# zuston/TonY

Hardware: AMD Instinct MI355X
Metric: images/sec (whole node) Inception-v3 TF-PS (higher is better)
Workload: dtype bf16

## Files before the change

tony_amd/ops/_lib.py:

```python
from __future__ import annotations

import ctypes
import os
import threading
import weakref
from typing import Dict

import torch

_HERE = os.path.dirname(os.path.abspath(__file__))
SO_PATH = os.environ.get("TONY_KERNELS_SO") or os.path.join(_HERE, "_tony_kernels.so")

_lock = threading.Lock()
_lib = None

c_void_p = ctypes.c_void_p
c_int = ctypes.c_int
c_int64 = ctypes.c_int64
c_float = ctypes.c_float
c_int_p = ctypes.POINTER(ctypes.c_int)
c_void_pp = ctypes.POINTER(ctypes.c_void_p)
c_u8_p = ctypes.POINTER(ctypes.c_uint8)
c_u64_p = ctypes.POINTER(ctypes.c_uint64)

_SIGNATURES = {
    "tony_bn_fwd_train": [c_void_p, c_int64, c_int, c_int64, c_void_p, c_int64, c_void_p, c_void_p, c_int,
                          c_float, c_int, c_void_p, c_void_p, c_void_p, c_void_p, c_void_p, c_float, c_void_p],
    "tony_bn_fwd_infer": [c_void_p, c_int64, c_int, c_int64, c_void_p, c_int64, c_void_p, c_void_p, c_int,
                          c_float, c_int, c_void_p, c_void_p, c_void_p],
    "tony_bn_bwd": [c_void_p, c_int64, c_void_p, c_int64, c_void_p, c_int64, c_int64, c_int, c_void_p, c_void_p,
                    c_void_p, c_void_p, c_int, c_int, c_void_p, c_void_p, c_void_p, c_int, c_void_p],
    "tony_stat_shards": [],
    "tony_bn_stats": [c_void_p, c_int64, c_int, c_int64, c_void_p, c_void_p, c_int64, c_void_p],
    "tony_bn_apply": [c_void_p, c_int64, c_int, c_int64, c_void_p, c_int64, c_void_p, c_void_p, c_int64, c_void_p,
                      c_void_p, c_int, c_float, c_int, c_int, c_void_p, c_void_p, c_void_p, c_void_p, c_float,
                      c_void_p],
    "tony_bn_apply_segs": [c_void_p, c_int64, c_int, c_int64, c_int, c_int, c_int, c_int, c_int, c_void_p, c_void_p,
                           c_void_p, c_void_p, c_int64, c_int64, c_int64, c_int64, c_void_p, c_void_p, c_int64,
                           c_void_p, c_void_p, c_int, c_float, c_int, c_int, c_void_p, c_void_p, c_void_p, c_void_p,
                           c_float, c_void_p],
    "tony_bn_bwd_reduce_segs": [c_void_p, c_int64, c_int, c_int, c_int, c_int, c_int, c_void_p, c_void_p, c_void_p,
                                c_void_p, c_int64, c_int64, c_int64, c_int64, c_int64, c_int, c_void_p, c_void_p,
                                c_void_p, c_void_p, c_int, c_int, c_void_p, c_void_p, c_int64, c_void_p],
    "tony_bn_bwd_apply_segs": [c_void_p, c_int64, c_int, c_int, c_int, c_int, c_int, c_void_p, c_void_p, c_void_p,
                               c_void_p, c_int64, c_int64, c_int64, c_int64, c_void_p, c_int64, c_int64, c_int,
                               c_void_p, c_void_p, c_void_p, c_void_p, c_int, c_int, c_void_p, c_void_p, c_int64,
                               c_void_p, c_void_p, c_int, c_void_p],
    "tony_bn_relu_maxpool": [c_void_p, c_int64, c_void_p, c_void_p, c_int64, c_void_p, c_void_p, c_int, c_float,
                             c_void_p, c_void_p, c_void_p, c_void_p, c_float, c_void_p, c_int64, c_void_p, c_int,
                             c_int, c_int, c_int, c_int, c_int, c_int, c_void_p],
    "tony_bn_bwd_reduce": [c_void_p, c_int64, c_void_p, c_int64, c_int64, c_int, c_void_p, c_void_p, c_void_p,
                           c_void_p, c_int, c_int, c_void_p, c_void_p, c_int64, c_void_p],
    "tony_bn_bwd_apply": [c_void_p, c_int64, c_void_p, c_int64, c_void_p, c_int64, c_int64, c_int, c_void_p,
                          c_void_p, c_void_p, c_void_p, c_int, c_int, c_void_p, c_void_p, c_int64, c_void_p,
                          c_void_p, c_int, c_void_p],
    "tony_bn_apply_f32_x3": [c_void_p, c_int64, c_int, c_int64, c_void_p, c_int64, c_void_p, c_void_p, c_int64,
                             c_void_p, c_void_p, c_int, c_float, c_int, c_int, c_void_p, c_void_p, c_void_p, c_void_p,
                             c_float, c_void_p],
    "tony_bn_apply_res": [c_void_p, c_int64, c_int, c_int64, c_void_p, c_int64, c_void_p, c_int64, c_void_p,
                          c_void_p, c_int64, c_void_p, c_void_p, c_int, c_float, c_int, c_int, c_void_p, c_void_p,
                          c_void_p, c_void_p, c_float, c_void_p],
    "tony_bn_apply_res_m": [c_void_p, c_int64, c_int, c_int64, c_void_p, c_int64, c_void_p, c_int64, c_void_p,
                            c_void_p, c_int64, c_void_p, c_void_p, c_int, c_float, c_int, c_int, c_void_p, c_void_p,
                            c_void_p, c_void_p, c_float, c_void_p, c_int64, c_void_p],
    "tony_bn_bwd_res": [c_void_p, c_int64, c_void_p, c_int64, c_void_p, c_int64, c_void_p, c_int64, c_void_p, c_int64,
                        c_int64, c_int, c_void_p, c_void_p, c_void_p, c_void_p, c_int, c_void_p, c_void_p, c_void_p,
                        c_int, c_void_p],
    "tony_bn_bwd_res_m": [c_void_p, c_int64, c_void_p, c_int64, c_void_p, c_int64, c_void_p, c_int64, c_void_p,
                          c_int64, c_int64, c_int, c_void_p, c_void_p, c_void_p, c_void_p, c_int, c_void_p, c_void_p,
                          c_void_p, c_int, c_void_p],
    "tony_bn_bwd_onepass": [c_void_p, c_int64, c_void_p, c_int64, c_void_p, c_int64, c_int64, c_int, c_void_p,
                            c_void_p, c_void_p, c_void_p, c_int, c_int, c_void_p, c_void_p, c_void_p, c_int,
                            c_void_p, c_int, c_void_p],
    "tony_add_f32": [c_void_p, c_int, c_void_p, c_int64, c_void_p],
    "tony_sgd_step": [c_void_p, c_void_p, c_void_p, c_int, c_void_p, c_int64, c_void_p, c_void_p],
    "tony_adam_step": [c_void_p, c_void_p, c_void_p, c_void_p, c_int, c_void_p, c_int64, c_void_p, c_void_p],
    "tony_adagrad_step": [c_void_p, c_void_p, c_void_p, c_int, c_void_p, c_int64, c_void_p, c_void_p],
    "tony_rmsprop_step": [c_void_p, c_void_p, c_void_p, c_void_p, c_int, c_void_p, c_int64, c_void_p, c_void_p],
    "tony_grad_stats": [c_void_p, c_int, c_int64, c_void_p, c_void_p],
    "tony_xent_fwd": [c_void_p, c_int, c_int64, c_int, c_int64, c_void_p, c_float, c_void_p, c_void_p, c_void_p],
    "tony_xent_bwd": [c_void_p, c_int, c_int64, c_int, c_int64, c_void_p, c_float, c_void_p, c_void_p, c_void_p,
                      c_int64, c_void_p],
    "tony_dropout_fwd": [c_void_p, c_void_p, c_void_p, c_int64, c_int, c_float, c_void_p, c_void_p],
    "tony_dropout_bwd": [c_void_p, c_void_p, c_void_p, c_int64, c_int, c_float, c_void_p],
    "tony_counter_bump": [c_void_p, c_void_p],
    "tony_gemm_bf16": [c_void_p, c_void_p, c_void_p, c_int64, c_int64, c_int64, c_int64, c_int64, c_int64,
                       c_int, c_void_p, c_int64, c_void_p],
    "tony_gemm_bf16_bnact": [c_void_p, c_void_p, c_void_p, c_int64, c_int64, c_int64, c_int64, c_int64, c_int64,
                             c_int, c_void_p, c_int64, c_void_p, c_void_p],
    "tony_gemm_tn_bf16": [c_void_p, c_void_p, c_void_p, c_int64, c_int64, c_int64, c_int64, c_int64, c_int64,
                          c_void_p, c_int64, c_void_p, c_int, c_void_p, c_void_p, c_int, c_void_p],
    "tony_splitk_reduce": [c_void_p, c_int, c_int64, c_void_p, c_int, c_int, c_int, c_void_p],
    "tony_splitk_workspace": [c_void_p, c_int64, c_void_p, c_int64],
    "tony_conv_fwd": [c_void_p, c_int, c_int, c_int, c_int, c_int64, c_void_p, c_int, c_int, c_int, c_int, c_int,
                      c_int, c_int, c_void_p, c_int, c_int, c_int64, c_int, c_void_p, c_int64, c_void_p],
    "tony_stem_fwd": [c_void_p, c_int, c_int, c_int, c_int, c_void_p, c_int, c_int, c_int, c_int, c_int, c_int,
                      c_int, c_void_p, c_int, c_int, c_int64, c_int, c_void_p, c_int64, c_int, c_void_p],
    "tony_stem_wgrad": [c_void_p, c_int64, c_void_p, c_int, c_int, c_int, c_int, c_int, c_int, c_int, c_int, c_int,
                        c_int, c_int, c_int, c_int, c_void_p, c_int64, c_void_p, c_int, c_void_p],
    "tony_conv_dgrad": [c_void_p, c_int, c_int, c_int, c_int, c_int64, c_void_p, c_int, c_int, c_int, c_int, c_int,
                        c_void_p, c_int, c_int, c_int64, c_int, c_void_p, c_void_p],
    "tony_conv_dgrad_strided": [c_void_p, c_int, c_int, c_int, c_int, c_int64, c_void_p, c_int, c_int, c_int, c_int,
                                c_int, c_int, c_int, c_void_p, c_int, c_int, c_int64, c_int, c_void_p, c_void_p],
    "tony_conv_wgrad": [c_void_p, c_int64, c_void_p, c_int, c_int, c_int, c_int, c_int64, c_int, c_int, c_int, c_int,
                        c_int, c_int, c_int, c_int, c_int, c_void_p, c_void_p, c_int64, c_void_p, c_int, c_void_p,
                        c_void_p, c_int, c_void_p],
    "tony_conv_wgrad_x3": [c_void_p, c_int64, c_void_p, c_int, c_int, c_int, c_int, c_int64, c_int, c_int, c_int,
                           c_int, c_int, c_int, c_int, c_int, c_int, c_int, c_int, c_void_p, c_int64, c_void_p, c_int,
                           c_void_p],
    "tony_x3_wgrad_mode": [c_int],
    "tony_dgrad_one_launch": [c_int],
    "tony_wgrad_pf": [c_int],
    "tony_kv_copy_blocks": [c_int64],
    "tony_kv_copy_flag": [c_void_p, c_void_p, c_int64, c_void_p, c_void_p],
    "tony_kv_wait": [c_void_p, ctypes.c_uint32, c_void_p, ctypes.c_double, c_void_p],
    "tony_conv_wgrad_direct": [c_void_p, c_int64, c_void_p, c_int, c_int, c_int, c_int, c_int64, c_int, c_int, c_int,
                               c_int, c_int, c_void_p, c_int64, c_void_p, c_int, c_void_p],
    "tony_avgpool3_s1p1": [c_void_p, c_void_p, c_int, c_int, c_int, c_int, c_int64, c_int64, c_void_p],
    "tony_maxpool_fwd": [c_void_p, c_void_p, c_void_p, c_int, c_int, c_int, c_int, c_int, c_int, c_int, c_int64, c_int64,
                         c_void_p],
    "tony_maxpool_bwd": [c_void_p, c_void_p, c_void_p, c_int, c_int, c_int, c_int, c_int, c_int, c_int, c_int64, c_int64,
                         c_void_p],
    "tony_bn_bwd_pool_apply": [c_void_p, c_int64, c_void_p, c_int, c_int, c_int, c_int, c_int, c_int, c_int, c_void_p,
                               c_int64, c_void_p, c_int64, c_void_p, c_void_p, c_void_p, c_void_p, c_int, c_int,
                               c_void_p, c_int64, c_void_p, c_void_p, c_int, c_void_p],
    "tony_maxpool_bwd_acc": [c_void_p, c_void_p, c_void_p, c_int, c_int, c_int, c_int, c_int, c_int, c_int, c_int64, c_int64,
                         c_void_p],
    "tony_maxpool_bwd_bnred": [c_void_p, c_void_p, c_void_p, c_int, c_int, c_int, c_int, c_int, c_int, c_int, c_int64,
                               c_int64, c_void_p, c_int64, c_void_p, c_void_p, c_void_p, c_void_p, c_int, c_int,
                               c_void_p, c_int64, c_int, c_void_p],
    "tony_avgpool_fwd": [c_void_p, c_void_p, c_int, c_int, c_int, c_int, c_int, c_int, c_int64, c_int64, c_void_p],
    "tony_avgpool_bwd": [c_void_p, c_void_p, c_int, c_int, c_int, c_int, c_int, c_int, c_int64, c_int64, c_void_p],
    "tony_transpose_desc_bytes": [],
    "tony_x3_desc_bytes": [],
    "tony_x3_weights_batch": [c_void_p, c_int, c_int, c_void_p],
    "tony_transpose_batch": [c_void_p, c_int, c_int, c_void_p],
    "tony_event_pool": [c_int, c_u64_p],
    "tony_fork": [c_void_p, c_void_p, c_void_p],
    "tony_bn_stats_f32": [c_void_p, c_int64, c_int, c_int64, c_void_p, c_void_p, c_int64, c_void_p],
    "tony_bn_apply_f32": [c_void_p, c_int64, c_int, c_int64, c_void_p, c_int64, c_void_p, c_void_p, c_int64, c_void_p,
                      c_void_p, c_int, c_float, c_int, c_int, c_void_p, c_void_p, c_void_p, c_void_p, c_float,
                      c_void_p],
    "tony_bn_bwd_reduce_f32": [c_void_p, c_int64, c_void_p, c_int64, c_int64, c_int, c_void_p, c_void_p, c_void_p,
                           c_void_p, c_int, c_int, c_void_p, c_void_p, c_int64, c_void_p],
    "tony_bn_bwd_apply_f32": [c_void_p, c_int64, c_void_p, c_int64, c_void_p, c_int64, c_int64, c_int, c_void_p,
                          c_void_p, c_void_p, c_void_p, c_int, c_int, c_void_p, c_void_p, c_int64, c_void_p,
                          c_void_p, c_int, c_void_p],
    "tony_bn_bwd_apply_f32_x3": [c_void_p, c_int64, c_void_p, c_int64, c_void_p, c_int64, c_int64, c_int, c_void_p,
                          c_void_p, c_void_p, c_void_p, c_int, c_int, c_void_p, c_void_p, c_int64, c_void_p,
                          c_void_p, c_int, c_void_p],
    "tony_bn_bwd_apply_f32_x3p": [c_void_p, c_int64, c_void_p, c_int64, c_void_p, c_int64, c_int64, c_int64, c_int,
                                  c_void_p, c_void_p, c_void_p, c_void_p, c_int, c_int, c_void_p, c_void_p, c_int64,
                                  c_void_p, c_void_p, c_int, c_void_p],
    "tony_avgpool3_s1p1_f32": [c_void_p, c_void_p, c_int, c_int, c_int, c_int, c_int64, c_int64, c_void_p],
    "tony_avgpool3_s1p1_x3p": [c_void_p, c_void_p, c_int, c_int, c_int, c_int, c_int64, c_int64, c_int64, c_void_p],
    "tony_avgpool3_s1p1_acc": [c_void_p, c_void_p, c_int, c_int, c_int, c_int, c_int64, c_int64, c_int, c_void_p],
    "tony_avgpool3_s1p1_x3": [c_void_p, c_void_p, c_int, c_int, c_int, c_int, c_int64, c_void_p],
    "tony_maxpool_fwd_f32": [c_void_p, c_void_p, c_void_p, c_int, c_int, c_int, c_int, c_int, c_int, c_int, c_int64, c_int64,
                         c_void_p],
    "tony_maxpool_bwd_f32": [c_void_p, c_void_p, c_void_p, c_int, c_int, c_int, c_int, c_int, c_int, c_int, c_int64, c_int64,
                         c_void_p],
    "tony_maxpool_bwd_acc_f32": [c_void_p, c_void_p, c_void_p, c_int, c_int, c_int, c_int, c_int, c_int, c_int, c_int64, c_int64,
                         c_void_p],
    "tony_avgpool_fwd_f32": [c_void_p, c_void_p, c_int, c_int, c_int, c_int, c_int, c_int, c_int64, c_int64, c_void_p],
    "tony_avgpool_bwd_f32": [c_void_p, c_void_p, c_int, c_int, c_int, c_int, c_int, c_int, c_int64, c_int64, c_void_p],
    "tony_x3_split": [c_void_p, c_int64, c_int64, c_int, c_int, c_void_p, c_int64, c_int, c_void_p],
    "tony_x3_split_slice": [c_void_p, c_int64, c_int64, c_int, c_void_p, c_int64, c_int, c_int, c_void_p],
    "tony_bn_apply_f32_p3": [c_void_p, c_int64, c_int, c_int64, c_void_p, c_int64, c_void_p, c_int64, c_int64,
                             c_void_p, c_void_p, c_int64, c_void_p, c_void_p, c_int, c_float, c_int, c_int, c_void_p,
                             c_void_p, c_void_p, c_void_p, c_float, c_void_p],
    "tony_x3_weights_t": [c_void_p, c_int, c_int, c_int, c_void_p, c_void_p],
    "tony_plan_mark": [c_int, c_void_p],
    "tony_plan_build": [c_void_p, c_u64_p, c_int, c_u64_p, c_int_p],
    "tony_plan_replay": [c_void_p, c_int, c_void_p],
    "tony_plan_segments": [c_void_p],
    "tony_plan_failure": [c_void_p, c_int_p],
    "tony_plan_ops": [c_void_p, c_int_p, c_int],
    "tony_plan_destroy": [c_void_p],
    "tony_ps_header_bytes": [],
    "tony_kv_copy": [c_void_p, c_void_p, c_int64, c_void_p, c_void_p],
    "tony_ps_max_buckets": [],
    "tony_ps_max_blocks": [],
    "tony_ps_land_entry_bytes": [],
    "tony_ps_window_alloc": [c_int64, c_void_pp, c_u8_p],
    "tony_ps_push": [c_void_p, c_int, c_void_p, c_int64, c_int, c_int64, c_int, c_int, ctypes.c_uint32, c_int,
                     c_void_p],
    "tony_ps_apply": [c_void_p, c_int64, c_int64, c_int, c_int, c_int64, c_int64, c_void_p, c_void_p, c_void_p,
                      c_void_p, c_int, c_u64_p, c_void_p, c_int, c_int, ctypes.c_uint32, c_int, ctypes.c_double,
                      c_int, c_void_p],
    "tony_ps_land": [c_void_p, c_void_p, c_int, c_void_p, c_int, ctypes.c_uint32, ctypes.c_double, c_void_p],
    "tony_ps_error_async": [c_void_p, c_void_p, c_void_p],
    "tony_ps_error": [c_void_p, c_int_p],
    "tony_xgmi_max_ranks": [],
    "tony_xgmi_handle_bytes": [],
    "tony_xgmi_alloc": [c_int64, c_void_pp, c_u8_p],
    "tony_xgmi_open": [c_u8_p, c_void_pp],
    "tony_xgmi_close": [c_void_p],
    "tony_xgmi_free": [c_void_p],
    "tony_xgmi_error": [c_void_p, c_int_p],
    "tony_xgmi_error_async": [c_void_p, c_void_p, c_void_p],
    "tony_xgmi_collective": [c_u64_p, c_int, c_int, c_int64, c_int, c_void_p, c_void_p, c_int64, c_int, c_int,
                             c_float, ctypes.c_uint32, c_int, c_void_p],
}


class BnRed(ctypes.Structure):
    _fields_ = [("z", c_void_p), ("ldz", c_int64), ("mean", c_void_p), ("invstd", c_void_p), ("gamma", c_void_p),
                ("beta", c_void_p), ("pb", c_int), ("relu", c_int), ("dsum", c_void_p), ("sstride", c_int64),
                ("done", c_int)]


class _SignedLib:

    def __init__(self, h):
        self._h = h
        for name, argtypes in _SIGNATURES.items():
            fn = getattr(h, name, None)
            if fn is None:
                continue
            fn.argtypes = argtypes
            fn.restype = c_int
            setattr(self, name, fn)
        self.fastcall = 0
        if os.environ.get("TONY_FASTCALL", "1") != "0":
            try:
                from . import _tony_fastcall, fastcall
            except ImportError:
                _tony_fastcall = None
            if _tony_fastcall is not None:
                for name, w in fastcall.bind_all(_tony_fastcall, h, _SIGNATURES).items():
                    setattr(self, name, w)
                    self.fastcall += 1
        set_ws = self.__dict__.get("tony_splitk_workspace")
        if set_ws is not None:
            for name, fpos in _SPLITK_ENTRIES.items():
                fn = self.__dict__.get(name)
                if fn is not None:
                    setattr(self, name, _splitk_entry(fn, set_ws, fpos))

    def __getattr__(self, name):
        raise KernelError(f"{name}: not exported by {SO_PATH} or missing from _lib._SIGNATURES")


class KernelError(RuntimeError):
    pass


_SPLITK_ENTRIES = {"tony_gemm_bf16": 9, "tony_conv_fwd": 18, "tony_conv_dgrad": 16}
SPLITK_MAX_TILES = 4096


def splitk_slab_floats(m: int, cus: int) -> int:
    return 2 * m * cus * 256 * 192


def _splitk_entry(fn, set_ws, fpos: int):
    def call(*a):
        s = (a[fpos] >> 16) & 15
        if not s:
            return fn(*a)
        from .arena import zeros_f32

        dev = torch.device("cuda", torch.cuda.current_device())
        slab = torch.empty(splitk_slab_floats(s, num_cus(dev)), dtype=torch.float32, device=dev)
        cnt = zeros_f32(2 * SPLITK_MAX_TILES, dev)
        check(set_ws(slab.data_ptr(), slab.numel(), cnt.data_ptr(), cnt.numel()), "tony_splitk_workspace")
        try:
            return fn(*a)
        finally:
            set_ws(0, 0, 0, 0)

    call.__name__ = getattr(fn, "__name__", "splitk_entry")
    call.__wrapped__ = fn
    return call


STAT_SHARDS = 8


def stat_floats(c: int) -> int:
    return STAT_SHARDS * 2 * c


def check_stat_buffer(buf, c: int) -> None:
    if buf is not None and (buf.dtype != torch.float32 or buf.numel() < stat_floats(c) or not buf.is_contiguous()):
        raise ValueError(f"statistics buffer for {c} channels must be {stat_floats(c)} contiguous fp32 "
                         f"(STAT_SHARDS={STAT_SHARDS} x [sum | sumsq]); got {buf.dtype} x {buf.numel()}")


BN_ONEPASS = os.environ.get("TONY_BN_ONEPASS", "0") == "1"
BN_ONEPASS_MAX_BYTES = int(os.environ.get("TONY_BN_ONEPASS_MAX_MB", "0")) << 20


def bn_bwd_ws_floats(c: int) -> int:
    return stat_floats(c) + 4


def bn_bwd(x, ldx: int, dy, lddy: int, dx, lddx: int, M: int, C: int, mean, invstd, gamma, beta, pb: int,
           relu: bool, ws, dgamma, dbeta, accumulate: bool, device, sums=None) -> None:
    L = lib()
    if sums is not None:
        rc = L.tony_bn_bwd_apply(x.data_ptr(), ldx, dy.data_ptr(), lddy, dx.data_ptr(), lddx, M, C, mean.data_ptr(),
                                 invstd.data_ptr(), ptr(gamma), ptr(beta), pb, int(relu), sums.data_ptr(),
                                 sums.data_ptr() + 4 * C, 2 * C, ptr(dgamma), ptr(dbeta), int(accumulate),
                                 stream_ptr(device))
        check(rc, "tony_bn_bwd_apply")
        return
    if BN_ONEPASS and ws.numel() >= stat_floats(C) + 1 and (BN_ONEPASS_MAX_BYTES == 0 or
                                                             2 * M * C <= BN_ONEPASS_MAX_BYTES):
        rc = L.tony_bn_bwd_onepass(x.data_ptr(), ldx, dy.data_ptr(), lddy, dx.data_ptr(), lddx, M, C,
                                   mean.data_ptr(), invstd.data_ptr(), ptr(gamma), ptr(beta), pb, int(relu),
                                   ws.data_ptr(), ptr(dgamma), ptr(dbeta), int(accumulate),
                                   ws.data_ptr() + 4 * stat_floats(C), num_cus(device), stream_ptr(device))
        check(rc, "tony_bn_bwd_onepass")
        return
    rc = L.tony_bn_bwd(x.data_ptr(), ldx, dy.data_ptr(), lddy, dx.data_ptr(), lddx, M, C, mean.data_ptr(),
                       invstd.data_ptr(), ptr(gamma), ptr(beta), pb, int(relu), ws.data_ptr(), ptr(dgamma), ptr(dbeta),
                       int(accumulate), stream_ptr(device))
    check(rc, "tony_bn_bwd")


def fold_stats(buf, c: int):
    return buf[:stat_floats(c)].view(STAT_SHARDS, 2 * c).sum(0)


def lib():
    global _lib
    if _lib is not None:
        return _lib
    with _lock:
        if _lib is not None:
            return _lib
        if not os.path.exists(SO_PATH):
            raise KernelError(
                f"{SO_PATH} is missing: run `python -m tony_amd.ops.build` (or __graft_entry__.build())")
        h = _SignedLib(ctypes.CDLL(SO_PATH, mode=ctypes.RTLD_LOCAL))
        n = h.tony_stat_shards()
        if n != STAT_SHARDS:
            raise KernelError(f"{SO_PATH} accumulates BN statistics in {n} shards, the Python side expects "
                              f"{STAT_SHARDS}: rebuild the kernels")
        _lib = h
    return _lib


def available() -> bool:
    try:
        lib()
        return True
    except (KernelError, OSError):
        return False


_RAW_STREAM = getattr(torch._C, "_cuda_getCurrentRawStream", None)


def stream_ptr(device=None) -> int:
    if _RAW_STREAM is not None:
        idx = getattr(device, "index", None)
        return _RAW_STREAM(torch.cuda.current_device() if idx is None else idx)
    return torch.cuda.current_stream(device).cuda_stream


def check(rc: int, name: str):
    if rc != 0:
        raise KernelError(f"{name} failed with code {rc}")


_NUM_CUS = {}


def num_cus(device) -> int:
    idx = device.index if device.index is not None else torch.cuda.current_device()
    if idx not in _NUM_CUS:
        _NUM_CUS[idx] = torch.cuda.get_device_properties(idx).multi_processor_count
    return _NUM_CUS[idx]


_INPLACE_GRADS = [True]


def set_inplace_grads(enabled: bool) -> None:
    _INPLACE_GRADS[0] = bool(enabled)


_SLOT_OK: Dict[int, tuple] = {}


def grad_slot(param):
    if not _INPLACE_GRADS[0] or param is None or not isinstance(param, torch.nn.Parameter):
        return None
    g = param.grad
    if g is None:
        return None
    hit = _SLOT_OK.get(id(param))
    if hit is not None and hit[0]() is g:
        return g if hit[1] else None
    ok = (g.dtype == param.dtype and g.shape == param.shape
          and (g.is_contiguous() or (g.dim() == 4 and g.is_contiguous(memory_format=torch.channels_last))))
    if len(_SLOT_OK) > 65536:
        _SLOT_OK.clear()
    _SLOT_OK[id(param)] = (weakref.ref(g), ok)
    return g if ok else None


_GRAD_LISTENERS: "weakref.WeakSet" = weakref.WeakSet()


def add_grad_listener(listener) -> None:
    _GRAD_LISTENERS.add(listener)


def remove_grad_listener(listener) -> None:
    _GRAD_LISTENERS.discard(listener)


def grads_ready(*params) -> None:
    if _GRAD_LISTENERS:
        ps = [p for p in params if p is not None]
        for lst in list(_GRAD_LISTENERS):
            lst.ready(ps)


def report_inplace(params, returned) -> None:
    if _GRAD_LISTENERS:
        grads_ready(*[p for p, g in zip(params, returned)
                      if g is None and isinstance(p, torch.nn.Parameter) and p.requires_grad])


def ptr(t) -> int:
    return 0 if t is None else t.data_ptr()


def check_f32_stats(*tensors) -> None:
    for t in tensors:
        if t is not None and t.dtype != torch.float32:
            raise TypeError(f"BatchNorm running statistics must be float32, got {t.dtype}; "
                            "cast models with tony_amd.models.layers.cast_model(model, dtype)")
```

tony_amd/ops/csrc/band.hip:

```cpp
#include <algorithm>

#include "igemm.h"

using namespace tony;
using namespace tony::mfma;
using namespace tony::glds;

namespace {

constexpr int kBandThreads = 512;
constexpr int kKC = 32;
constexpr int kAP = kKC + 16;
constexpr int kBM = 256;
constexpr int kMaxHaloPx = 512;
constexpr int kNA = kMaxHaloPx * (kKC / 8) / kBandThreads;

struct BandArgs {
  const uint16_t* src;
  int64_t ld;
  const uint16_t* B;
  uint16_t* C;
  int64_t ldc;
  float* stats;
  int64_t sstride;
  int N, Cs;
  int lines, per_img;
  int wd, hp, L;
  int h0;
  int win;
  int64_t s_img, s_line, s_pos;
  int64_t o_img, o_line, o_pos;
  int sign;
  int ntn;
};

template <int T, int BN>
__global__ __launch_bounds__(kBandThreads) void conv_band_kernel(BandArgs a) {
  constexpr int BP = T * kKC + 16;
  constexpr int TN = BN / 32;
  constexpr int NB = (BN * T * (kKC / 8) + kBandThreads - 1) / kBandThreads;
  extern __shared__ __attribute__((aligned(16))) uint16_t bsm[];
  const int hpx = a.L * a.hp;
  uint16_t* ha = bsm;
  uint16_t* hb = bsm + hpx * kAP;

  const int tn = blockIdx.x % a.ntn;
  const int tm = blockIdx.x / a.ntn;
  const int line0 = tm * a.L, n0 = tn * BN;
  const int lane = threadIdx.x & 63, wave = threadIdx.x >> 6;
  const int wm = wave & 3, wn = wave >> 2;
  const int kq = lane >> 4;

  int64_t asrc[kNA];
  int adst[kNA];
#pragma unroll
  for (int i = 0; i < kNA; ++i) {
    const int v = i * kBandThreads + threadIdx.x;
    const int px = v >> 2, c8 = v & 3;
    asrc[i] = -1;
    adst[i] = -1;
    if (px < hpx) {
      const int ln = px / a.hp, p = px - ln * a.hp;
      const int gl = line0 + ln, sp = a.h0 + p;
      adst[i] = px * kAP + c8 * 8;
      if (gl < a.lines && static_cast<unsigned>(sp) < static_cast<unsigned>(a.win)) {
        const int img = gl / a.per_img, li = gl - img * a.per_img;
        asrc[i] = img * a.s_img + li * a.s_line + sp * a.s_pos + c8 * 8;
      }
    }
  }
  int64_t bsrc[NB];
  int bdst[NB];
#pragma unroll
  for (int i = 0; i < NB; ++i) {
    const int v = i * kBandThreads + threadIdx.x;
    const int row = v / (T * 4), rem = v - row * (T * 4);
    const int t = rem >> 2, c8 = rem & 3;
    bsrc[i] = -1;
    bdst[i] = -1;
    if (row < BN) {
      bdst[i] = row * BP + t * kKC + c8 * 8;
      if (n0 + row < a.N) bsrc[i] = static_cast<int64_t>(n0 + row) * T * a.Cs + t * a.Cs + c8 * 8;
    }
  }
  uint4 ra[kNA], rb[NB];
  auto fetch = [&](int c0) {
#pragma unroll
    for (int i = 0; i < kNA; ++i)
      ra[i] = asrc[i] >= 0 ? *reinterpret_cast<const uint4*>(a.src + asrc[i] + c0) : make_uint4(0u, 0u, 0u, 0u);
#pragma unroll
    for (int i = 0; i < NB; ++i)
      rb[i] = bsrc[i] >= 0 ? *reinterpret_cast<const uint4*>(a.B + bsrc[i] + c0) : make_uint4(0u, 0u, 0u, 0u);
  };
  auto stage = [&]() {
#pragma unroll
    for (int i = 0; i < kNA; ++i)
      if (adst[i] >= 0) *reinterpret_cast<uint4*>(ha + adst[i]) = ra[i];
#pragma unroll
    for (int i = 0; i < NB; ++i)
      if (bdst[i] >= 0) *reinterpret_cast<uint4*>(hb + bdst[i]) = rb[i];
  };

  int abase[4];
#pragma unroll
  for (int i = 0; i < 4; ++i) {
    const int m = wm * 64 + i * 16 + (lane & 15);
    const int ln = m / a.wd, p = m - ln * a.wd;
    abase[i] = (m < a.L * a.wd ? ln * a.hp + p : 0) * kAP + kq * 8;
  }
  f32x4 acc[4][TN];
#pragma unroll
  for (int i = 0; i < 4; ++i)
#pragma unroll
    for (int j = 0; j < TN; ++j) acc[i][j] = f32x4{0.f, 0.f, 0.f, 0.f};

  const int nchunks = a.Cs / kKC;
  fetch(0);
  for (int ch = 0; ch < nchunks; ++ch) {
    __syncthreads();
    stage();
    __syncthreads();
    if (ch + 1 < nchunks) fetch((ch + 1) * kKC);
#pragma unroll
    for (int t = 0; t < T; ++t) {
      const int tt = a.sign > 0 ? t : T - 1 - t;
      bf16x8_t af[4], bfr[TN];
#pragma unroll
      for (int i = 0; i < 4; ++i) af[i] = *reinterpret_cast<const bf16x8_t*>(ha + abase[i] + tt * kAP);
#pragma unroll
      for (int j = 0; j < TN; ++j)
        bfr[j] = *reinterpret_cast<const bf16x8_t*>(hb + (wn * (BN / 2) + j * 16 + (lane & 15)) * BP + t * kKC + kq * 8);
#pragma unroll
      for (int i = 0; i < 4; ++i)
#pragma unroll
        for (int j = 0; j < TN; ++j) acc[i][j] = __builtin_amdgcn_mfma_f32_16x16x32_bf16(af[i], bfr[j], acc[i][j], 0, 0, 0);
    }
  }

  bool rv[4][4];
#pragma unroll
  for (int i = 0; i < 4; ++i)
#pragma unroll
    for (int q = 0; q < 4; ++q) {
      const int m = wm * 64 + i * 16 + kq * 4 + q;
      rv[i][q] = m < a.L * a.wd && line0 + m / a.wd < a.lines;
    }
  if (a.stats != nullptr) {
    float* st = a.stats + shard_off(blockIdx.x, a.sstride);
#pragma unroll
    for (int j = 0; j < TN; ++j) {
      const int col = n0 + wn * (BN / 2) + j * 16 + (lane & 15);
      float sm = 0.f, sq = 0.f;
#pragma unroll
      for (int i = 0; i < 4; ++i)
#pragma unroll
        for (int q = 0; q < 4; ++q) {
          const float v = rv[i][q] ? acc[i][j][q] : 0.f;
          sm += v;
          sq = fmaf(v, v, sq);
        }
      sm += __shfl_xor(sm, 16, 64);
      sm += __shfl_xor(sm, 32, 64);
      sq += __shfl_xor(sq, 16, 64);
      sq += __shfl_xor(sq, 32, 64);
      if (lane < 16 && col < a.N) {
        atomicAdd(st + col, sm);
        atomicAdd(st + a.N + col, sq);
      }
    }
  }
  __syncthreads();
  constexpr int LDC = BN + 8;
  uint16_t* cs = bsm;
#pragma unroll
  for (int i = 0; i < 4; ++i)
#pragma unroll
    for (int j = 0; j < TN; ++j)
#pragma unroll
      for (int q = 0; q < 4; ++q)
        cs[(wm * 64 + i * 16 + kq * 4 + q) * LDC + wn * (BN / 2) + j * 16 + (lane & 15)] = f2bf(acc[i][j][q]);
  __syncthreads();
  for (int v = threadIdx.x; v < kBM * (BN / 8); v += kBandThreads) {
    const int m = v / (BN / 8), c8 = v - m * (BN / 8);
    if (m >= a.L * a.wd || n0 + c8 * 8 >= a.N) continue;
    const int ln = m / a.wd, p = m - ln * a.wd;
    const int gl = line0 + ln;
    if (gl >= a.lines) continue;
    const int img = gl / a.per_img, li = gl - img * a.per_img;
    uint16_t* dst = a.C + img * a.o_img + li * a.o_line + p * a.o_pos + n0 + c8 * 8;
    *reinterpret_cast<uint4*>(dst) = *reinterpret_cast<const uint4*>(cs + m * LDC + c8 * 8);
  }
}

template <int T, int BN>
int launch_band(const BandArgs& a, int grid, hipStream_t stream) {
  constexpr size_t kMaxLds = (static_cast<size_t>(kMaxHaloPx) * kAP + static_cast<size_t>(BN) * (T * kKC + 16)) * 2;
  static_assert(kMaxLds <= 163840, "LDS");
  const size_t lds = std::max((static_cast<size_t>(a.L) * a.hp * kAP + static_cast<size_t>(BN) * (T * kKC + 16)) * 2,
                              static_cast<size_t>(kBM) * (BN + 8) * 2);
  const void* fn = reinterpret_cast<const void*>(&conv_band_kernel<T, BN>);
  static int ok = 0;
  if (ok == 0)
    ok = hipFuncSetAttribute(fn, hipFuncAttributeMaxDynamicSharedMemorySize, static_cast<int>(kMaxLds)) == hipSuccess
             ? 1
             : -1;
  if (ok < 0 || lds > kMaxLds) return -3;
  conv_band_kernel<T, BN><<<grid, kBandThreads, lds, stream>>>(a);
  TONY_LAUNCH_CHECK();
  return 0;
}

}

namespace tony {

int run_band(const Gather& g, const void* B, void* C, int64_t ldc, int64_t N, int epi, float* st, int64_t sstride,
             hipStream_t stream) {
  if ((epi & ~1) || ((epi & 1) && st == nullptr) || g.sh != 1 || g.sw != 1 || (g.Cs % kKC) || (g.ld % 8) ||
      (ldc % 8) || N <= 0 || N > 0x7fffffff || g.halo_images <= 0 || (reinterpret_cast<uintptr_t>(C) & 15) ||
      (reinterpret_cast<uintptr_t>(B) & 15) || (reinterpret_cast<uintptr_t>(g.src) & 15))
    return -3;
  const bool along_w = g.R == 1 && g.S > 1;
  const bool along_h = g.S == 1 && g.R > 1;
  if (!along_w && !along_h) return -3;
  const int T = along_w ? g.S : g.R;
  if (T != 3 && T != 7) return -3;
  BandArgs a{};
  a.src = static_cast<const uint16_t*>(g.src);
  a.ld = g.ld;
  a.B = static_cast<const uint16_t*>(B);
  a.C = static_cast<uint16_t*>(C);
  a.ldc = ldc;
  a.stats = (epi & 1) ? st : nullptr;
  a.sstride = sstride;
  a.N = static_cast<int>(N);
  a.Cs = g.Cs;
  a.sign = g.sign;
  a.s_img = static_cast<int64_t>(g.Hs) * g.Ws * g.ld;
  a.o_img = static_cast<int64_t>(g.OH) * g.OW * ldc;
  if (along_w) {
    if (g.offh != 0 || g.Hs != g.OH) return -3;
    a.per_img = g.OH;
    a.wd = g.OW;
    a.win = g.Ws;
    a.h0 = g.offw + (g.sign < 0 ? -(T - 1) : 0);
    a.s_line = static_cast<int64_t>(g.Ws) * g.ld;
    a.s_pos = g.ld;
    a.o_line = static_cast<int64_t>(g.OW) * ldc;
    a.o_pos = ldc;
  } else {
    if (g.offw != 0 || g.Ws != g.OW) return -3;
    a.per_img = g.OW;
    a.wd = g.OH;
    a.win = g.Hs;
    a.h0 = g.offh + (g.sign < 0 ? -(T - 1) : 0);
    a.s_line = g.ld;
    a.s_pos = static_cast<int64_t>(g.Ws) * g.ld;
    a.o_line = ldc;
    a.o_pos = static_cast<int64_t>(g.OW) * ldc;
  }
  a.hp = a.wd + T - 1;
  a.L = kBM / a.wd;
  if (a.L < 1 || a.L * a.hp > kMaxHaloPx) return -3;
  const int64_t lines = static_cast<int64_t>(g.halo_images) * a.per_img;
  if (lines > 0x7fffffff) return -2;
  a.lines = static_cast<int>(lines);
  const int bn = (N % 96 == 0) ? 96 : 64;
  a.ntn = static_cast<int>((N + bn - 1) / bn);
  const int64_t grid = (lines + a.L - 1) / a.L * a.ntn;
  if (grid > 0x7fffffff) return -2;
  if (T == 7) return bn == 96 ? launch_band<7, 96>(a, static_cast<int>(grid), stream)
                              : launch_band<7, 64>(a, static_cast<int>(grid), stream);
  return bn == 96 ? launch_band<3, 96>(a, static_cast<int>(grid), stream)
                  : launch_band<3, 64>(a, static_cast<int>(grid), stream);
}

}
```

Before: 9662.

## Pipeline band conv kernel with async global-to-LDS loads and multi-buffered halos

Rewrites the 1xT/Tx1 band convolution kernel to stream input halos and filter slices straight from global memory into LDS through direct async loads. Halos are multi-buffered and filter slices use a 4-stage ring, replacing the old register-staged, double-synchronised loop. The change also adds XOR swizzling to avoid LDS bank conflicts, raises MFMA priority with s_setprio, and picks per-T tile sizes with N tiles of 128/160/192. The goal is to overlap memory latency with MFMA work and cut barrier stalls. The cost is much more complex synchronisation and occupancy that now depends on LDS use, and N tiles can waste work when N is not a multiple of the tile.

```diff
diff --git a/tony_amd/ops/_lib.py b/tony_amd/ops/_lib.py
--- a/tony_amd/ops/_lib.py
+++ b/tony_amd/ops/_lib.py
@@ -111,6 +111,7 @@
     "tony_x3_wgrad_mode": [c_int],
     "tony_dgrad_one_launch": [c_int],
     "tony_wgrad_pf": [c_int],
+    "tony_band_geometry": [c_int, c_int, c_int64, c_int],
     "tony_kv_copy_blocks": [c_int64],
     "tony_kv_copy_flag": [c_void_p, c_void_p, c_int64, c_void_p, c_void_p],
     "tony_kv_wait": [c_void_p, ctypes.c_uint32, c_void_p, ctypes.c_double, c_void_p],
diff --git a/tony_amd/ops/csrc/band.hip b/tony_amd/ops/csrc/band.hip
--- a/tony_amd/ops/csrc/band.hip
+++ b/tony_amd/ops/csrc/band.hip
@@ -9,11 +9,24 @@
 namespace {
 
 constexpr int kBandThreads = 512;
+constexpr int kBandWaves = kBandThreads / 64;
 constexpr int kKC = 32;
-constexpr int kAP = kKC + 16;
-constexpr int kBM = 256;
-constexpr int kMaxHaloPx = 512;
-constexpr int kNA = kMaxHaloPx * (kKC / 8) / kBandThreads;
+constexpr int kNS = 4;
+constexpr int kHaloPad = 8;
+#ifndef TONY_BAND_PRIO
+#define TONY_BAND_PRIO 1
+#endif
+constexpr bool kBandPrio = TONY_BAND_PRIO != 0;
+constexpr int kLgkm0 = 0xc07f;
+
+template <int T>
+struct BandCfg {
+  static constexpr int BM = T == 7 ? 256 : 128;
+  static constexpr int NH = T == 7 ? 2 : 4;
+  static constexpr int CAP = T == 7 ? 512 : 256;
+  static_assert(T - 1 <= kHaloPad, "halo pad");
+  static_assert(((NH - 1) * T + 1) / 2 >= kNS, "a halo buffer's last read precedes its refill (WAR)");
+};
 
 struct BandArgs {
   const uint16_t* src;
@@ -32,119 +45,173 @@
   int64_t o_img, o_line, o_pos;
   int sign;
   int ntn;
+  int hbytes;
 };
+
+__device__ __forceinline__ int band_sw(int r) { return ((r >> 2) & 1) << 1; }
 
 template <int T, int BN>
 __global__ __launch_bounds__(kBandThreads) void conv_band_kernel(BandArgs a) {
-  constexpr int BP = T * kKC + 16;
+  using Cfg = BandCfg<T>;
+  constexpr int BM = Cfg::BM, NH = Cfg::NH, NS = kNS;
+  constexpr int TM = BM / 64;
   constexpr int TN = BN / 32;
-  constexpr int NB = (BN * T * (kKC / 8) + kBandThreads - 1) / kBandThreads;
+  constexpr int GB = 2 * BN * 64;
+  constexpr int GI = 2 * BN / 16;
+  constexpr int NBI = (GI + kBandWaves - 1) / kBandWaves;
+  constexpr int NHI = Cfg::CAP / 16 / kBandWaves;
+  static_assert(BN % 32 == 0 && NS >= 3, "tile shape");
   extern __shared__ __attribute__((aligned(16))) uint16_t bsm[];
-  const int hpx = a.L * a.hp;
-  uint16_t* ha = bsm;
-  uint16_t* hb = bsm + hpx * kAP;
 
   const int tn = blockIdx.x % a.ntn;
   const int tm = blockIdx.x / a.ntn;
   const int line0 = tm * a.L, n0 = tn * BN;
-  const int lane = threadIdx.x & 63, wave = threadIdx.x >> 6;
+  const int lane = threadIdx.x & 63, wave = __builtin_amdgcn_readfirstlane(threadIdx.x >> 6);
   const int wm = wave & 3, wn = wave >> 2;
   const int kq = lane >> 4;
-
-  int64_t asrc[kNA];
-  int adst[kNA];
-#pragma unroll
-  for (int i = 0; i < kNA; ++i) {
-    const int v = i * kBandThreads + threadIdx.x;
-    const int px = v >> 2, c8 = v & 3;
+  const int hpx = a.L * a.hp;
+  const int nhp = (hpx + 15) >> 4;
+  const uint32_t lbase = __builtin_amdgcn_readfirstlane(lds_addr(bsm));
+  const uint32_t fbase = lbase + NH * a.hbytes;
+  const uint16_t* zc = reinterpret_cast<const uint16_t*>(&kZeroChunk);
+
+  int64_t asrc[NHI];
+#pragma unroll
+  for (int i = 0; i < NHI; ++i) {
+    const int px = (wave + kBandWaves * i) * 16 + (lane >> 2);
+    const int c8 = (lane & 3) ^ band_sw(px);
+    const int ln = px / a.hp, p = px - ln * a.hp;
+    const int gl = line0 + ln, sp = a.h0 + p;
     asrc[i] = -1;
-    adst[i] = -1;
-    if (px < hpx) {
-      const int ln = px / a.hp, p = px - ln * a.hp;
-      const int gl = line0 + ln, sp = a.h0 + p;
-      adst[i] = px * kAP + c8 * 8;
-      if (gl < a.lines && static_cast<unsigned>(sp) < static_cast<unsigned>(a.win)) {
-        const int img = gl / a.per_img, li = gl - img * a.per_img;
-        asrc[i] = img * a.s_img + li * a.s_line + sp * a.s_pos + c8 * 8;
+    if (px < hpx && p < a.wd + T - 1 && gl < a.lines && static_cast<unsigned>(sp) < static_cast<unsigned>(a.win)) {
+      const int img = gl / a.per_img, li = gl - img * a.per_img;
+      asrc[i] = img * a.s_img + li * a.s_line + sp * a.s_pos + c8 * 8;
+    }
+  }
+  int64_t bsrc[NBI];
+  int bq[NBI];
+#pragma unroll
+  for (int i = 0; i < NBI; ++i) {
+    bq[i] = min(wave + kBandWaves * i, GI - 1);
+    const int rr = bq[i] * 16 + (lane >> 2);
+    const int row = rr % BN;
+    const int c8 = (lane & 3) ^ band_sw(row);
+    bsrc[i] = n0 + row < a.N ? static_cast<int64_t>(n0 + row) * T * a.Cs + c8 * 8 : -1;
+  }
+  const int nchunks = a.Cs / kKC;
+  const int nsl = nchunks * T;
+  const int ng = (nsl + 1) >> 1;
+
+  auto issue_group = [&](int gi) {
+    const int s0 = gi * 2;
+    const int c = (s0 + T - 1) / T;
+    if (c * T <= s0 + 1 && c < nchunks) {
+      const uint32_t hb = lbase + (c % NH) * a.hbytes;
+#pragma unroll
+      for (int i = 0; i < NHI; ++i) {
+        const int q = wave + kBandWaves * i;
+        if (q < nhp) glds16(asrc[i] >= 0 ? a.src + asrc[i] + c * kKC : zc, hb + q * 1024);
       }
     }
-  }
-  int64_t bsrc[NB];
-  int bdst[NB];
-#pragma unroll
-  for (int i = 0; i < NB; ++i) {
-    const int v = i * kBandThreads + threadIdx.x;
-    const int row = v / (T * 4), rem = v - row * (T * 4);
-    const int t = rem >> 2, c8 = rem & 3;
-    bsrc[i] = -1;
-    bdst[i] = -1;
-    if (row < BN) {
-      bdst[i] = row * BP + t * kKC + c8 * 8;
-      if (n0 + row < a.N) bsrc[i] = static_cast<int64_t>(n0 + row) * T * a.Cs + t * a.Cs + c8 * 8;
-    }
-  }
-  uint4 ra[kNA], rb[NB];
-  auto fetch = [&](int c0) {
-#pragma unroll
-    for (int i = 0; i < kNA; ++i)
-      ra[i] = asrc[i] >= 0 ? *reinterpret_cast<const uint4*>(a.src + asrc[i] + c0) : make_uint4(0u, 0u, 0u, 0u);
-#pragma unroll
-    for (int i = 0; i < NB; ++i)
-      rb[i] = bsrc[i] >= 0 ? *reinterpret_cast<const uint4*>(a.B + bsrc[i] + c0) : make_uint4(0u, 0u, 0u, 0u);
+    const uint32_t fs = fbase + (gi % NS) * GB;
+    int64_t so[2];
+#pragma unroll
+    for (int k = 0; k < 2; ++k) {
+      const int s = s0 + k, ch = s / T, t = s - ch * T;
+      so[k] = s < nsl ? static_cast<int64_t>(t) * a.Cs + ch * kKC : -1;
+    }
+#pragma unroll
+    for (int i = 0; i < NBI; ++i) {
+      const int64_t o = bq[i] * 16 >= BN ? so[1] : so[0];
+      glds16(bsrc[i] >= 0 && o >= 0 ? a.B + bsrc[i] + o : zc, fs + bq[i] * 1024);
+    }
   };
-  auto stage = [&]() {
-#pragma unroll
-    for (int i = 0; i < kNA; ++i)
-      if (adst[i] >= 0) *reinterpret_cast<uint4*>(ha + adst[i]) = ra[i];
-#pragma unroll
-    for (int i = 0; i < NB; ++i)
-      if (bdst[i] >= 0) *reinterpret_cast<uint4*>(hb + bdst[i]) = rb[i];
+
+  int apix[TM];
+#pragma unroll
+  for (int i = 0; i < TM; ++i) {
+    const int m = wm * (BM / 4) + i * 16 + (lane & 15);
+    const int ln = m / a.wd, p = m - ln * a.wd;
+    apix[i] = m < a.L * a.wd ? ln * a.hp + p : 0;
+  }
+  int boff[TN];
+#pragma unroll
+  for (int j = 0; j < TN; ++j) {
+    const int n = wn * (BN / 2) + j * 16 + (lane & 15);
+    boff[j] = n * 64 + ((kq ^ band_sw(n)) << 4);
+  }
+  f32x4 acc[TM][TN];
+#pragma unroll
+  for (int i = 0; i < TM; ++i)
+#pragma unroll
+    for (int j = 0; j < TN; ++j) acc[i][j] = f32x4{0.f, 0.f, 0.f, 0.f};
+
+  const uint8_t* lds = reinterpret_cast<const uint8_t*>(bsm);
+  const uint8_t* fl = lds + NH * a.hbytes;
+  auto rd = [&](bf16x8_t (&af)[TM], bf16x8_t (&bfr)[TN], int slot, int k, int ch, int t) {
+    const int tt = a.sign > 0 ? t : T - 1 - t;
+    const uint8_t* hb = lds + (ch % NH) * a.hbytes;
+#pragma unroll
+    for (int i = 0; i < TM; ++i) {
+      const int px = apix[i] + tt;
+      af[i] = *reinterpret_cast<const bf16x8_t*>(hb + px * 64 + ((kq ^ band_sw(px)) << 4));
+    }
+    const uint8_t* fb = fl + slot * GB + k * (BN * 64);
+#pragma unroll
+    for (int j = 0; j < TN; ++j) bfr[j] = *reinterpret_cast<const bf16x8_t*>(fb + boff[j]);
   };
-
-  int abase[4];
-#pragma unroll
-  for (int i = 0; i < 4; ++i) {
-    const int m = wm * 64 + i * 16 + (lane & 15);
-    const int ln = m / a.wd, p = m - ln * a.wd;
-    abase[i] = (m < a.L * a.wd ? ln * a.hp + p : 0) * kAP + kq * 8;
-  }
-  f32x4 acc[4][TN];
-#pragma unroll
-  for (int i = 0; i < 4; ++i)
-#pragma unroll
-    for (int j = 0; j < TN; ++j) acc[i][j] = f32x4{0.f, 0.f, 0.f, 0.f};
-
-  const int nchunks = a.Cs / kKC;
-  fetch(0);
-  for (int ch = 0; ch < nchunks; ++ch) {
-    __syncthreads();
-    stage();
-    __syncthreads();
-    if (ch + 1 < nchunks) fetch((ch + 1) * kKC);
-#pragma unroll
-    for (int t = 0; t < T; ++t) {
-      const int tt = a.sign > 0 ? t : T - 1 - t;
-      bf16x8_t af[4], bfr[TN];
-#pragma unroll
-      for (int i = 0; i < 4; ++i) af[i] = *reinterpret_cast<const bf16x8_t*>(ha + abase[i] + tt * kAP);
-#pragma unroll
-      for (int j = 0; j < TN; ++j)
-        bfr[j] = *reinterpret_cast<const bf16x8_t*>(hb + (wn * (BN / 2) + j * 16 + (lane & 15)) * BP + t * kKC + kq * 8);
-#pragma unroll
-      for (int i = 0; i < 4; ++i)
-#pragma unroll
-        for (int j = 0; j < TN; ++j) acc[i][j] = __builtin_amdgcn_mfma_f32_16x16x32_bf16(af[i], bfr[j], acc[i][j], 0, 0, 0);
-    }
-  }
-
-  bool rv[4][4];
-#pragma unroll
-  for (int i = 0; i < 4; ++i)
-#pragma unroll
-    for (int q = 0; q < 4; ++q) {
-      const int m = wm * 64 + i * 16 + kq * 4 + q;
-      rv[i][q] = m < a.L * a.wd && line0 + m / a.wd < a.lines;
-    }
+  auto mm = [&](const bf16x8_t (&af)[TM], const bf16x8_t (&bfr)[TN]) {
+    if (kBandPrio) __builtin_amdgcn_s_setprio(1);
+#pragma unroll
+    for (int i = 0; i < TM; ++i)
+#pragma unroll
+      for (int j = 0; j < TN; ++j) acc[i][j] = __builtin_amdgcn_mfma_f32_16x16x32_bf16(af[i], bfr[j], acc[i][j], 0, 0, 0);
+    if (kBandPrio) __builtin_amdgcn_s_setprio(0);
+  };
+
+  for (int gi = 0; gi < NS && gi < ng; ++gi) issue_group(gi);
+  if (NS - 1 < ng) glds_wait_barrier<(NS - 1) * NBI>();
+  else glds_wait_barrier<0>();
+  int slot = 0, ch = 0, t = 0;
+  bf16x8_t af0[TM], bf0[TN], af1[TM], bf1[TN];
+  rd(af0, bf0, 0, 0, 0, 0);
+  __builtin_amdgcn_s_waitcnt(kLgkm0);
+  for (int g = 0; g < ng; ++g) {
+    int ch1 = ch, t1 = t + 1;
+    if (t1 == T) {
+      t1 = 0;
+      ++ch1;
+    }
+    const bool odd = ch1 == nchunks;
+    rd(af1, bf1, slot, 1, odd ? nchunks - 1 : ch1, odd ? (a.sign > 0 ? 0 : T - 1) : t1);
+    mm(af0, bf0);
+    ch = ch1;
+    t = t1 + 1;
+    if (t == T) {
+      t = 0;
+      ++ch;
+    }
+    const int nslot = slot + 1 == NS ? 0 : slot + 1;
+    __builtin_amdgcn_sched_barrier(0);
+    __builtin_amdgcn_s_waitcnt(kLgkm0);
+    if (g + 1 < ng) {
+      if (g + NS - 1 < ng) glds_wait_barrier<(NS - 2) * NBI>();
+      else glds_wait_barrier<0>();
+      if (g + NS < ng) issue_group(g + NS);
+      rd(af0, bf0, nslot, 0, ch, t);
+    }
+    mm(af1, bf1);
+    __builtin_amdgcn_sched_barrier(0);
+    __builtin_amdgcn_s_waitcnt(kLgkm0);
+    slot = nslot;
+  }
+
+  const int mvalid = min(a.L, a.lines - line0) * a.wd;
+  bool rv[TM][4];
+#pragma unroll
+  for (int i = 0; i < TM; ++i)
+#pragma unroll
+    for (int q = 0; q < 4; ++q) rv[i][q] = wm * (BM / 4) + i * 16 + kq * 4 + q < mvalid;
   if (a.stats != nullptr) {
     float* st = a.stats + shard_off(blockIdx.x, a.sstride);
 #pragma unroll
@@ -152,7 +219,7 @@
       const int col = n0 + wn * (BN / 2) + j * 16 + (lane & 15);
       float sm = 0.f, sq = 0.f;
 #pragma unroll
-      for (int i = 0; i < 4; ++i)
+      for (int i = 0; i < TM; ++i)
 #pragma unroll
         for (int q = 0; q < 4; ++q) {
           const float v = rv[i][q] ? acc[i][j][q] : 0.f;
@@ -173,46 +240,80 @@
   constexpr int LDC = BN + 8;
   uint16_t* cs = bsm;
 #pragma unroll
-  for (int i = 0; i < 4; ++i)
+  for (int i = 0; i < TM; ++i)
 #pragma unroll
     for (int j = 0; j < TN; ++j)
 #pragma unroll
       for (int q = 0; q < 4; ++q)
-        cs[(wm * 64 + i * 16 + kq * 4 + q) * LDC + wn * (BN / 2) + j * 16 + (lane & 15)] = f2bf(acc[i][j][q]);
+        cs[(wm * (BM / 4) + i * 16 + kq * 4 + q) * LDC + wn * (BN / 2) + j * 16 + (lane & 15)] = f2bf(acc[i][j][q]);
   __syncthreads();
-  for (int v = threadIdx.x; v < kBM * (BN / 8); v += kBandThreads) {
-    const int m = v / (BN / 8), c8 = v - m * (BN / 8);
-    if (m >= a.L * a.wd || n0 + c8 * 8 >= a.N) continue;
-    const int ln = m / a.wd, p = m - ln * a.wd;
-    const int gl = line0 + ln;
-    if (gl >= a.lines) continue;
-    const int img = gl / a.per_img, li = gl - img * a.per_img;
-    uint16_t* dst = a.C + img * a.o_img + li * a.o_line + p * a.o_pos + n0 + c8 * 8;
-    *reinterpret_cast<uint4*>(dst) = *reinterpret_cast<const uint4*>(cs + m * LDC + c8 * 8);
-  }
-}
+  constexpr int CPR = BN / 8, RPP = kBandThreads / CPR;
+  const int c8 = threadIdx.x % CPR;
+  int m = threadIdx.x / CPR;
+  if (m < RPP && n0 + c8 * 8 < a.N) {
+    int ln = m / a.wd, p = m - ln * a.wd;
+    int img = (line0 + ln) / a.per_img, li = line0 + ln - img * a.per_img;
+    const int dl = RPP / a.wd, dp = RPP - dl * a.wd;
+    for (; m < mvalid; m += RPP) {
+      uint16_t* dst = a.C + img * a.o_img + li * a.o_line + p * a.o_pos + n0 + c8 * 8;
+      *reinterpret_cast<uint4*>(dst) = *reinterpret_cast<const uint4*>(cs + m * LDC + c8 * 8);
+      p += dp;
+      li += dl;
+      if (p >= a.wd) {
+        p -= a.wd;
+        ++li;
+      }
+      while (li >= a.per_img) {
+        li -= a.per_img;
+        ++img;
+      }
+    }
+  }
+}
+
+constexpr size_t kBandMaxLds = 163840;
 
 template <int T, int BN>
 int launch_band(const BandArgs& a, int grid, hipStream_t stream) {
-  constexpr size_t kMaxLds = (static_cast<size_t>(kMaxHaloPx) * kAP + static_cast<size_t>(BN) * (T * kKC + 16)) * 2;
-  static_assert(kMaxLds <= 163840, "LDS");
-  const size_t lds = std::max((static_cast<size_t>(a.L) * a.hp * kAP + static_cast<size_t>(BN) * (T * kKC + 16)) * 2,
-                              static_cast<size_t>(kBM) * (BN + 8) * 2);
+  using Cfg = BandCfg<T>;
+  static_assert(static_cast<size_t>(Cfg::NH) * Cfg::CAP * 64 + static_cast<size_t>(kNS) * 2 * BN * 64 <= kBandMaxLds, "LDS");
+  const size_t lds = std::max(static_cast<size_t>(Cfg::NH) * a.hbytes + static_cast<size_t>(kNS) * 2 * BN * 64,
+                              static_cast<size_t>(Cfg::BM) * (BN + 8) * 2);
   const void* fn = reinterpret_cast<const void*>(&conv_band_kernel<T, BN>);
   static int ok = 0;
   if (ok == 0)
-    ok = hipFuncSetAttribute(fn, hipFuncAttributeMaxDynamicSharedMemorySize, static_cast<int>(kMaxLds)) == hipSuccess
+    ok = hipFuncSetAttribute(fn, hipFuncAttributeMaxDynamicSharedMemorySize, static_cast<int>(kBandMaxLds)) == hipSuccess
              ? 1
              : -1;
-  if (ok < 0 || lds > kMaxLds) return -3;
+  if (ok < 0 || lds > kBandMaxLds) return -3;
   conv_band_kernel<T, BN><<<grid, kBandThreads, lds, stream>>>(a);
   TONY_LAUNCH_CHECK();
   return 0;
 }
 
+template <int T>
+int launch_band_n(const BandArgs& a, int bn, int grid, hipStream_t stream) {
+  return bn == 128 ? launch_band<T, 128>(a, grid, stream)
+                   : bn == 160 ? launch_band<T, 160>(a, grid, stream) : launch_band<T, 192>(a, grid, stream);
+}
+
 }
 
 namespace tony {
+
+extern "C" int tony_band_geometry(int T, int wd, int64_t N, int what) {
+  if ((T != 3 && T != 7) || wd < 1 || N < 1) return 0;
+  const int BM = T == 7 ? BandCfg<7>::BM : BandCfg<3>::BM;
+  const int CAP = T == 7 ? BandCfg<7>::CAP : BandCfg<3>::CAP;
+  const int NH = T == 7 ? BandCfg<7>::NH : BandCfg<3>::NH;
+  const int hp = wd + kHaloPad;
+  const int L = std::min(BM / wd, CAP / hp);
+  if (L < 1) return 0;
+  const int bn = N <= 128 ? 128 : N <= 160 ? 160 : 192;
+  const size_t hbytes = static_cast<size_t>((L * hp + 15) / 16) * 1024;
+  const size_t lds = std::max(NH * hbytes + static_cast<size_t>(kNS) * 2 * bn * 64, static_cast<size_t>(BM) * (bn + 8) * 2);
+  return what == 0 ? BM : what == 1 ? L : what == 2 ? bn : static_cast<int>(lds);
+}
 
 int run_band(const Gather& g, const void* B, void* C, int64_t ldc, int64_t N, int epi, float* st, int64_t sstride,
              hipStream_t stream) {
@@ -259,20 +360,19 @@
     a.o_line = ldc;
     a.o_pos = static_cast<int64_t>(g.OW) * ldc;
   }
-  a.hp = a.wd + T - 1;
-  a.L = kBM / a.wd;
-  if (a.L < 1 || a.L * a.hp > kMaxHaloPx) return -3;
+  a.L = a.wd < 1 ? 0 : tony_band_geometry(T, a.wd, N, 1);
+  if (a.L < 1) return -3;
+  const int bn = tony_band_geometry(T, a.wd, N, 2);
+  a.hp = a.wd + kHaloPad;
+  a.hbytes = (a.L * a.hp + 15) / 16 * 1024;
   const int64_t lines = static_cast<int64_t>(g.halo_images) * a.per_img;
   if (lines > 0x7fffffff) return -2;
   a.lines = static_cast<int>(lines);
-  const int bn = (N % 96 == 0) ? 96 : 64;
   a.ntn = static_cast<int>((N + bn - 1) / bn);
   const int64_t grid = (lines + a.L - 1) / a.L * a.ntn;
   if (grid > 0x7fffffff) return -2;
-  if (T == 7) return bn == 96 ? launch_band<7, 96>(a, static_cast<int>(grid), stream)
-                              : launch_band<7, 64>(a, static_cast<int>(grid), stream);
-  return bn == 96 ? launch_band<3, 96>(a, static_cast<int>(grid), stream)
-                  : launch_band<3, 64>(a, static_cast<int>(grid), stream);
-}
-
-}
+  return T == 7 ? launch_band_n<7>(a, bn, static_cast<int>(grid), stream)
+                : launch_band_n<3>(a, bn, static_cast<int>(grid), stream);
+}
+
+}
```

After: 9432. 0.976x the previous value.
